# nv-tlabs/NKSR

Hardware: AMD Instinct MI355X
Metric: reconstructed points/sec (solve+mesh) (higher is better)
Workload: dtype f32

## Files before the change

nksr_amd/csrc/fused_sweep.hip:

```cpp
#include "fused_dev.h"
#include <type_traits>

__device__ __forceinline__ int half_lane_i(int v, int l, bool upper) {
    const int lo = __builtin_amdgcn_readlane(v, l), hi = __builtin_amdgcn_readlane(v, 32 + l);
    return upper ? hi : lo;
}
__device__ __forceinline__ float half_lane_f(float v, int l, bool upper) { return __int_as_float(half_lane_i(__float_as_int(v), l, upper)); }

template <bool SETUP> struct FzSets { static constexpr int N = SETUP ? 2 : 1, SECOND = N - 1; };

template <int D, bool SETUP> struct FzStage { static constexpr int CAP0 = SETUP ? 64 : 96, CAP1 = D > 1 ? (SETUP ? 16 : 32) : 1; };
template <int D, bool SETUP> using FzStaged0 = float[FzSets<SETUP>::N][FzStage<D, SETUP>::CAP0 * 27];
template <int D, bool SETUP> using FzStaged1 = float[FzSets<SETUP>::N][FzStage<D, SETUP>::CAP1 * 27];
#define FZ_RCAP 288
template <int D, bool FAC = true> struct FzRecords {
    static constexpr int RS = FZ_RCAP + 4 * FZ_HW;
    float4 fv[FAC ? D * RS : 1], fp[FAC ? RS : 1];
};

template <int D, bool SETUP>
__device__ __forceinline__ void fz_zero_uncovered(const FusedArgs& A, int W0, float* __restrict__ part, float* __restrict__ part2) {
    if (W0 > 0 && threadIdx.x < 32 * D) {
        const int d = threadIdx.x >> 5;
        const int c = A.row_cells[(int64_t)d * A.rows_total + W0 - 1];
        if (c >= 0 && A.nbr32[(int64_t)c * 32 + 29] >= W0) {
            const int64_t blk = (int64_t)A.nbr32[(int64_t)c * 32 + 27] + blockIdx.x;
            part[blk * 32 + (threadIdx.x & 31)] = 0.f;
            if (SETUP) part2[blk * 32 + (threadIdx.x & 31)] = 0.f;
        }
    }
    if (SETUP && A.nnz_counter && threadIdx.x == 0) A.nnz_counter[1 + blockIdx.x] = 0;
}

template <int D, bool SETUP>
__device__ __forceinline__ void fz_flush(const FzStaged0<D, SETUP>& st0, const FzStaged1<D, SETUP>& st1, const int* stf, float* __restrict__ ct,
                                         float* __restrict__ ct2, int cw0, int cw1, int M) {
    constexpr int SECOND = FzSets<SETUP>::SECOND, CAP0 = FzStage<D, SETUP>::CAP0, CAP1 = FzStage<D, SETUP>::CAP1;
    const int t = threadIdx.x;
    const bool l0 = t < CAP0, l1 = !l0 && t < CAP0 + CAP1;
    if ((l0 || l1) && stf[t]) {
        const float* src = l0 ? st0[0] + t * 27 : st1[0] + (t - CAP0) * 27;
        const float* srcb = SETUP ? (l0 ? st0[SECOND] + t * 27 : st1[SECOND] + (t - CAP0) * 27) : nullptr;
        float* dst = ct + (l0 ? cw0 + t : cw1 + (t - CAP0));
        float* dstb = SETUP ? ct2 + (l0 ? cw0 + t : cw1 + (t - CAP0)) : nullptr;
#pragma unroll
        for (int q = 0; q < 27; ++q) {
            dst[(int64_t)q * M] = src[q];
            if (SETUP) dstb[(int64_t)q * M] = srcb[q];
        }
    }
}

struct FzSpline { float a[3], b[3], c[3]; };
__device__ __forceinline__ FzSpline fz_spline_consts(int s) {
    FzSpline q;
    const int o[3] = {s / 9, (s / 3) % 3, s % 3};
#pragma unroll
    for (int ax = 0; ax < 3; ++ax) {
        q.a[ax] = o[ax] == 1 ? 0.75f : 0.f;
        q.b[ax] = o[ax] == 1 ? -1.f : 0.5f;
        q.c[ax] = o[ax] == 0 ? 1.f : (o[ax] == 1 ? 0.5f : 0.f);
    }
    return q;
}
template <bool DER>
__device__ __forceinline__ void fz_axis(float p, float scale, float a, float b, float c, float k, float& w, float& dw) {
    const float u = __builtin_amdgcn_fractf(p * scale);
    const float t = u - c, bt = b * t;
    w = fmaf(bt, t, a);
    if (DER) dw = bt * k;
}
__device__ __forceinline__ float fz_dot4(const float4& a, const float4& b) {
    return fmaf(a.w, b.w, fmaf(a.z, b.z, fmaf(a.y, b.y, a.x * b.x)));
}

template <int D>
__device__ __forceinline__ void fz_stage_records(const FusedArgs& A, int W0, int W1, FzRecords<D>& R) {
    const int nw = W1 - W0 < FZ_RCAP ? W1 - W0 : FZ_RCAP;
    if (nw > 0) {
        const int t0 = threadIdx.x, t1 = threadIdx.x + FZ_BLOCK;
        float4 v0[D + 1], v1[D + 1];
#pragma unroll
        for (int d = 0; d <= D; ++d) {
            const float4* src = (d < D ? A.fac_vec + (int64_t)d * A.rows_total : A.fac_pos) + W0;
            v0[d] = src[t0 < nw ? t0 : nw - 1];
            v1[d] = src[t1 < nw ? t1 : nw - 1];
        }
        const float4 zero = make_float4(0.f, 0.f, 0.f, 0.f);
#pragma unroll
        for (int d = 0; d <= D; ++d) {
            float4* dst = d < D ? R.fv + d * R.RS : R.fp;
            if (t0 < nw + 4 && t0 < FZ_RCAP) dst[t0] = t0 < nw ? v0[d] : zero;
            if (t1 < nw + 4 && t1 < FZ_RCAP) dst[t1] = t1 < nw ? v1[d] : zero;
        }
    }
}

template <int D, bool SETUP>
__device__ __forceinline__ void fz_rebuild_rows(const FusedArgs& A, FzRecords<D>& R, const FzSpline& bq, float4 (&ps)[D], bool live0, const float4& pg,
                                                int r, int W0, int hwi, int s, bool act, int& nt, float (&w)[FZ_TRIP][D]) {
    constexpr int U = FZ_TRIP, RS = FzRecords<D>::RS;
    int rl = r - W0;
    if (rl + U > FZ_RCAP) {
        rl = FZ_RCAP + 4 * hwi;
        if (s < 4) {
            R.fp[rl + s] = A.fac_pos[(int64_t)r + s];
#pragma unroll
            for (int d = 0; d < D; ++d) R.fv[d * RS + rl + s] = A.fac_vec[(int64_t)d * A.rows_total + r + s];
        }
        __builtin_amdgcn_wave_barrier();
    }
    float4 pq[U];
#pragma unroll
    for (int u = 0; u < U; ++u) pq[u] = R.fp[rl + u];
    const bool site = __float_as_int(pq[0].w) == 1;
    const bool q1 = __float_as_int(pq[1].w) == 0, q2 = q1 && __float_as_int(pq[2].w) == 0, q3 = q2 && __float_as_int(pq[3].w) == 0;
    const int np = site ? U : 1 + (q1 ? 1 : 0) + (q2 ? 1 : 0) + (q3 ? 1 : 0);
    nt = nt < np ? nt : np;
    ps[0] = live0 ? pg : make_float4(0.f, 0.f, 0.f, 0.f);
#pragma unroll
    for (int d = 0; d < D; ++d) {
        const float scale = __int_as_float((127 - d) << 23);
        const float k2 = 2.f * A.inv_w0 * scale;
        float4 vq[U];
#pragma unroll
        for (int u = 0; u < U; ++u) vq[u] = R.fv[d * RS + rl + u];
        if (site) {
            float wx, wy, wz, dx, dy, dz;
            fz_axis<true>(pq[0].x, scale, bq.a[0], bq.b[0], bq.c[0], k2, wx, dx);
            fz_axis<true>(pq[0].y, scale, bq.a[1], bq.b[1], bq.c[1], k2, wy, dy);
            fz_axis<true>(pq[0].z, scale, bq.a[2], bq.b[2], bq.c[2], k2, wz, dz);
            const float yz = wy * wz, B = wx * yz;
            const float g = fz_dot4(vq[0], ps[d]);
            w[0][d] = 0.f;
            w[1][d] = fmaf(fz_dot4(vq[1], ps[d]), B, g * (dx * yz));
            w[2][d] = fmaf(fz_dot4(vq[2], ps[d]), B, g * ((wx * wz) * dy));
            w[3][d] = fmaf(fz_dot4(vq[3], ps[d]), B, g * ((wx * wy) * dz));
        } else {
#pragma unroll
            for (int u = 0; u < U; ++u) {
                float wx, wy, wz, unused;
                fz_axis<false>(pq[u].x, scale, bq.a[0], bq.b[0], bq.c[0], 0.f, wx, unused);
                fz_axis<false>(pq[u].y, scale, bq.a[1], bq.b[1], bq.c[1], 0.f, wy, unused);
                fz_axis<false>(pq[u].z, scale, bq.a[2], bq.b[2], bq.c[2], 0.f, wz, unused);
                w[u][d] = fz_dot4(vq[u], ps[d]) * (wx * (wy * wz));
            }
        }
    }
    if (SETUP && A.dense_out) {
#pragma unroll
        for (int d = 0; d < D; ++d)
            if (d >= A.dense_from && act)
#pragma unroll
                for (int u = 0; u < U; ++u)
                    if (u < nt) A.dense_out[((int64_t)(d - A.dense_from) * A.rows_total + r + u) * 27 + s] = w[u][d];
    }
}

template <int MODE, int D, bool FAC>
__global__ void __attribute__((amdgpu_waves_per_eu(FAC ? 3 : (D <= 4 ? 6 : 5)))) __launch_bounds__(FZ_BLOCK) k_fz_cells(FusedArgs A, const float* __restrict__ x, float* __restrict__ part,
                                                      float* __restrict__ part2, float* __restrict__ ct, float* __restrict__ ct2,
                                                      const int* __restrict__ done) {
    if (done && *done) return;
    constexpr bool SETUP = MODE == 1;
    constexpr int U = FZ_TRIP, SECOND = FzSets<SETUP>::SECOND;
    __shared__ float xv[FzSets<SETUP>::N][FZ_HW][D][2][32];
    __shared__ int xm[FZ_HW][D][2];
    __shared__ int xmb[FZ_HW][D][2];
    __shared__ int xbase[FZ_HW][D];
    __shared__ int wnnz[FZ_BLOCK / 64];
    constexpr int CAP0 = FzStage<D, SETUP>::CAP0, CAP1 = FzStage<D, SETUP>::CAP1;
    __shared__ FzStaged0<D, SETUP> st0;
    __shared__ FzStaged1<D, SETUP> st1;
    __shared__ int stf[CAP0 + CAP1];
    __shared__ FzRecords<D, FAC> R;
    for (int i = threadIdx.x; i < CAP0 + CAP1; i += FZ_BLOCK) stf[i] = 0;
    const int W0 = __builtin_amdgcn_readfirstlane(A.item_begin[blockIdx.x * FZ_HW]);
    if (__builtin_amdgcn_readfirstlane(A.item_begin[(blockIdx.x + 1) * FZ_HW]) == W0) {
        fz_zero_uncovered<D, SETUP>(A, W0, part, part2);
        return;
    }
    if constexpr (FAC) {
        const int W1 = __builtin_amdgcn_readfirstlane(A.item_begin[(blockIdx.x + 1) * FZ_HW]);
        if (MODE == 0 && W1 > W0 && fz_seg_done(A, A.item_seg, W0 >> 5)) return;
        fz_stage_records<D>(A, W0, W1, R);
    }
    __syncthreads();
    const int hwi = threadIdx.x >> 5;
    const int item = blockIdx.x * FZ_HW + hwi;
    const int s = threadIdx.x & 31;
    const bool act = s < 27, upper = (threadIdx.x & 32) != 0;
    const int sh = upper ? 32 : 0;
    const int sc = act ? s : 26;
    const int Rb = A.item_begin[item];
    int Re = A.item_begin[item + 1];
    if (MODE == 0 && Re > Rb && fz_seg_done(A, A.item_seg, Rb >> 5)) Re = Rb;
    const int cw0 = __builtin_amdgcn_readfirstlane((int64_t)W0 < A.rows_total ? A.row_cells[W0] : -1);
    const int cw1 = __builtin_amdgcn_readfirstlane((D > 1 && (int64_t)W0 < A.rows_total) ? A.row_cells[A.rows_total + W0] : -1);
    if (s < 2 * D) xm[hwi][s >> 1][s & 1] = -1;
    const int len32 = Re - Rb < 32 ? Re - Rb : 32;
    int cells[D];
    unsigned chg[D > 1 ? D : 2];
    unsigned um = 0;
#pragma unroll
    for (int d = 0; d < D; ++d) {
        cells[d] = s < len32 ? A.row_cells[(int64_t)d * A.rows_total + Rb + s] : -1;
        const int before = __shfl_up(cells[d], 1, 32);
        const unsigned m = (unsigned)(__ballot(s > 0 && s < len32 && cells[d] != before) >> sh);
        if (d > 0) chg[d] = m;
        um |= m;
    }
    um |= 1u;
    unsigned inside = 0;
    float P[FzSets<SETUP>::N][D], xs[D];
    bool have[D];
#pragma unroll
    for (int d = 0; d < D; ++d) { P[0][d] = 0.f; P[SECOND][d] = 0.f; xs[d] = 0.f; have[d] = false; }
    auto enter = [&](int d, int nbv) {
        const int first = __shfl(nbv, 28, 32), last = __shfl(nbv, 29, 32);
        if (s == 27) xbase[hwi][d] = nbv;
        inside = (inside & ~(3u << (2 * d))) | ((first >= Rb ? 1u : 0u) << (2 * d)) | ((last < Re ? 2u : 0u) << (2 * d));
    };
    auto finish = [&](int d, int cell, float p, float p2) {
        const int rel = d == 0 ? cell - cw0 : cell - cw1;
        if (d == 0 && cw0 >= 0 && (unsigned)rel < (unsigned)CAP0) {
            if (act) { st0[0][rel * 27 + s] = p; if (SETUP) st0[SECOND][rel * 27 + s] = p2; }
            if (s == 0) stf[rel] = 1;
        } else if (d == 1 && cw1 >= 0 && (unsigned)rel < (unsigned)CAP1) {
            if (act) { st1[0][rel * 27 + s] = p; if (SETUP) st1[SECOND][rel * 27 + s] = p2; }
            if (s == 0) stf[CAP0 + rel] = 1;
        } else if (act) {
            ct[(int64_t)s * A.M + cell] = p;
            if (SETUP) ct2[(int64_t)s * A.M + cell] = p2;
        }
    };
    auto emit = [&](int d, int cell, float p, float p2) {
        const unsigned f = (inside >> (2 * d)) & 3u;
        if (f == 3u) {
            finish(d, cell, p, p2);
        } else {
            const int k = (int)(f & 1u);
            xv[0][hwi][d][k][s] = p;
            if (SETUP) xv[SECOND][hwi][d][k][s] = p2;
            if (s == 0) { xm[hwi][d][k] = cell | ((f & 2u) ? (1 << 30) : 0); xmb[hwi][d][k] = xbase[hwi][d]; }
        }
    };
    auto unit_end = [&](int p) {
        const unsigned after = um & ~((2u << p) - 1u);
        return after ? Rb + (int)__builtin_ctz(after) : Re;
    };
    bool work = Rb < Re;
    int pos = 0, r = Rb, uend = unit_end(0);
    const float* wp[D];
#pragma unroll
    for (int d = 0; d < D; ++d) wp[d] = FAC ? nullptr : A.rows_all + (int64_t)d * A.rows_total * 27 + sc;
    int c0 = __shfl(cells[0], 0, 32);
    int line0;
    const float4 zero4 = make_float4(0.f, 0.f, 0.f, 0.f);
    float4 ps[D];
    {
        int cd[D], nb0[D];
        float x0[D];
        float4 p0[D];
#pragma unroll
        for (int d = 0; d < D; ++d) {
            cd[d] = __shfl(cells[d], 0, 32);
            nb0[d] = A.nbr32[(int64_t)(cd[d] >= 0 ? cd[d] : 0) * 32 + s];
        }
#pragma unroll
        for (int d = 1; d < D; ++d) {
            x0[d] = MODE == 0 ? x[(act && nb0[d] >= 0) ? nb0[d] : 0] : 0.f;
            if (FAC) p0[d] = A.psi_all[(act && nb0[d] >= 0) ? nb0[d] : 0];
        }
        line0 = nb0[0];
#pragma unroll
        for (int d = 1; d < D; ++d) {
            have[d] = work && cd[d] >= 0;
            enter(d, nb0[d]);
            xs[d] = (have[d] && act && nb0[d] >= 0) ? x0[d] : 0.f;
            if (FAC) ps[d] = (have[d] && act && nb0[d] >= 0) ? p0[d] : zero4;
        }
        if (FAC) ps[0] = zero4;
    }
    const FzSpline bq = fz_spline_consts(sc);
    int nnz = 0;
    while (__any(work)) {
        float w[U][D];
        if (!FAC) {
#pragma unroll
            for (int u = 0; u < U; ++u)
#pragma unroll
                for (int d = 0; d < D; ++d) w[u][d] = *(wp[d] + ((int64_t)r + u) * 27);
        }
        const float xg = MODE == 0 ? x[(act && line0 >= 0) ? line0 : 0] : 0.f;
        float4 pg = zero4;
        if (FAC) pg = A.psi_all[(act && line0 >= 0) ? line0 : 0];
        float tg[U];
        if (MODE == 1) {
#pragma unroll
            for (int u = 0; u < U; ++u) tg[u] = A.targets_all ? A.targets_all[r + u] : 0.f;
        }
        const int npos = uend - Rb;
        const int cn = __shfl(cells[0], npos & 31, 32);
        const int line0n = A.nbr32[(int64_t)((uend < Re && cn >= 0) ? cn : 0) * 32 + s];
        int nt = work ? (uend - r < U ? uend - r : U) : 0;
        if constexpr (FAC) {
            fz_rebuild_rows<D, SETUP>(A, R, bq, ps, c0 >= 0 && act && line0 >= 0, pg, r, W0, hwi, s, act, nt, w);
        }
        const float x0 = (c0 >= 0 && act && line0 >= 0) ? xg : 0.f;
        float t[U];
        if (MODE == 0) {
            float prod[U];
#pragma unroll
            for (int u = 0; u < U; ++u) {
                prod[u] = w[u][0] * x0;
#pragma unroll
                for (int d = 1; d < D; ++d) prod[u] = fmaf(w[u][d], xs[d], prod[u]);
            }
            const float rs = half_sum4(prod[0], prod[1], prod[2], prod[3], s);
#pragma unroll
            for (int u = 0; u < U; ++u) t[u] = u < nt ? half_lane_f(rs, 8 * u, upper) : 0.f;
        } else {
#pragma unroll
            for (int u = 0; u < U; ++u) {
                const bool ok = u < nt && act;
                t[u] = u < nt ? tg[u] : 0.f;
#pragma unroll
                for (int d = 0; d < D; ++d) { w[u][d] = ok ? w[u][d] : 0.f; nnz += w[u][d] != 0.f ? 1 : 0; }
            }
        }
#pragma unroll
        for (int u = 0; u < U; ++u)
#pragma unroll
            for (int d = 0; d < D; ++d) {
                P[0][d] = fmaf(w[u][d], t[u], P[0][d]);
                if (SETUP) P[SECOND][d] = fmaf(w[u][d], w[u][d], P[SECOND][d]);
            }
        r += nt;
        if (work && r >= uend) {
            if (c0 >= 0) finish(0, c0, P[0][0], P[SECOND][0]);
            P[0][0] = 0.f;
            if (SETUP) P[SECOND][0] = 0.f;
            work = uend < Re;
            if (work) {
                pos = npos;
                c0 = cn;
                line0 = line0n;
                uend = unit_end(pos);
#pragma unroll
                for (int d = 1; d < D; ++d)
                    if ((chg[d] >> pos) & 1u) {
                        const int before = __shfl(cells[d], (pos + 31) & 31, 32);
                        if (have[d]) emit(d, before, P[0][d], P[SECOND][d]);
                        P[0][d] = 0.f;
                        if (SETUP) P[SECOND][d] = 0.f;
                        xs[d] = 0.f;
                        if (FAC) ps[d] = zero4;
                        const int cd = __shfl(cells[d], pos, 32);
                        have[d] = cd >= 0;
                        if (have[d]) {
                            const int nbv = A.nbr32[(int64_t)cd * 32 + s];
                            enter(d, nbv);
                            if (MODE == 0 && act && nbv >= 0) xs[d] = x[nbv];
                            if (FAC && act && nbv >= 0) ps[d] = A.psi_all[nbv];
                        }
                    }
            }
        }
    }
#pragma unroll
    for (int d = 1; d < D; ++d)
        if (have[d]) emit(d, __shfl(cells[d], pos, 32), P[0][d], P[SECOND][d]);
    if (SETUP && A.nnz_counter) {
#pragma unroll
        for (int o = 32; o > 0; o >>= 1) nnz += __shfl_xor(nnz, o);
        if ((threadIdx.x & 63) == 0) wnnz[threadIdx.x >> 6] = nnz;
    }
    __syncthreads();
    if (SETUP && A.nnz_counter && threadIdx.x == 0) {
        unsigned long long tot = 0;
#pragma unroll
        for (int q = 0; q < FZ_BLOCK / 64; ++q) tot += (unsigned long long)wnnz[q];
        A.nnz_counter[1 + blockIdx.x] = tot;
    }
#pragma unroll
    for (int d = 1; d < D; ++d)
#pragma unroll
        for (int k = 0; k < 2; ++k) {
            const int e = xm[hwi][d][k];
            if (e < 0) continue;
            const int c = e & ~(1 << 30);
            const bool ends = (e >> 30) & 1;
            bool later = false;
            if (!ends)
                for (int h = hwi + 1; h < FZ_HW; ++h) later = later || (xm[h][d][0] >= 0 && (xm[h][d][0] & ~(1 << 30)) == c);
            if (later) continue;
            int h0 = hwi;
            bool started = k == 1;
            while (!started && h0 > 0) {
                --h0;
                started = xm[h0][d][1] >= 0 && (xm[h0][d][1] & ~(1 << 30)) == c;
            }
            float acc = 0.f, acc2 = 0.f;
            for (int h = h0; h <= hwi; ++h) {
                const int kk = (h == h0 && started) ? 1 : 0;
                const int eh = h == hwi ? e : xm[h][d][kk];
                if (eh < 0 || (eh & ~(1 << 30)) != c) continue;
                acc += xv[0][h][d][kk][s];
                if (SETUP) acc2 += xv[SECOND][h][d][kk][s];
            }
            if (started && ends) {
                finish(d, c, acc, acc2);
            } else {
                const int base = xmb[hwi][d][k];
                part[((int64_t)base + blockIdx.x) * 32 + s] = acc;
                if (SETUP) part2[((int64_t)base + blockIdx.x) * 32 + s] = acc2;
            }
        }
    __syncthreads();
    fz_flush<D, SETUP>(st0, st1, stf, ct, ct2, cw0, cw1, A.M);
}

template <int MAX, class F>
static inline void fz_with_depth(int depth, F&& f) {
    if constexpr (MAX > 1) {
        if (depth < MAX) return fz_with_depth<MAX - 1>(depth, f);
    }
    f(std::integral_constant<int, MAX>{});
}

template <int MODE>
void fz_sweep(const FusedArgs& A, const float* x, const FusedWork& w, const int* done, hipStream_t st) {
    if (A.hw_total <= 0) return;
    const dim3 grid(nksr_blocks((int64_t)A.hw_total, FZ_HW)), blk(FZ_BLOCK);
    fz_with_depth<NKSR_MAX_DEPTH>(A.depth, [&](auto depth) {
        constexpr int D = decltype(depth)::value;
        if (A.fac_vec) hipLaunchKernelGGL((k_fz_cells<MODE, D, true>), grid, blk, 0, st, A, x, w.part, w.part2, w.ct, w.ct2, done);
        else hipLaunchKernelGGL((k_fz_cells<MODE, D, false>), grid, blk, 0, st, A, x, w.part, w.part2, w.ct, w.ct2, done);
    });
}
template void fz_sweep<0>(const FusedArgs&, const float*, const FusedWork&, const int*, hipStream_t);
template void fz_sweep<1>(const FusedArgs&, const float*, const FusedWork&, const int*, hipStream_t);
```

Baseline: 33.25 million.

## Prefetch row weight tiles through a register ring staged via LDS in fz_cells

For the non-factored path, each half-wave now loads contiguous 16-byte pieces covering a trip's rows into a two-deep register ring, one trip ahead. It scatters them into an LDS tile and reads the per-lane weights back, replacing strided scalar global loads. Neighbour lines, x stencil values and targets are also fetched one trip ahead. Occupancy hints are lowered (waves_per_eu 6/5 to 4/3) to leave room for the extra live registers. The costs are more register pressure, more LDS use and explicit waitcnt/wave barriers, plus some risk in the row-advance bookkeeping at unit boundaries.

```diff
diff --git a/nksr_amd/csrc/fused_sweep.hip b/nksr_amd/csrc/fused_sweep.hip
--- a/nksr_amd/csrc/fused_sweep.hip
+++ b/nksr_amd/csrc/fused_sweep.hip
@@ -17,6 +17,18 @@
     static constexpr int RS = FZ_RCAP + 4 * FZ_HW;
     float4 fv[FAC ? D * RS : 1], fp[FAC ? RS : 1];
 };
+
+#define FZ_PIECES 28
+#define FZ_RING 2
+typedef float fz_piece_t __attribute__((ext_vector_type(4)));
+template <int D, bool ON = true> struct FzRowTiles { fz_piece_t v[ON ? FZ_HW * D * FZ_PIECES : 1]; };
+__device__ __forceinline__ const fz_piece_t* fz_row_piece(const float* rows, int64_t first, int s) {
+    const float* b = rows + first;
+    const int o4 = (int)(reinterpret_cast<uintptr_t>(b) & 12u);
+    int off = 16 * s < 428 + o4 ? 16 * s : 428 + o4;
+    off &= ~15;
+    return reinterpret_cast<const fz_piece_t*>(b + ((off - o4) >> 2));
+}
 
 template <int D, bool SETUP>
 __device__ __forceinline__ void fz_zero_uncovered(const FusedArgs& A, int W0, float* __restrict__ part, float* __restrict__ part2) {
@@ -158,7 +170,7 @@
 }
 
 template <int MODE, int D, bool FAC>
-__global__ void __attribute__((amdgpu_waves_per_eu(FAC ? 3 : (D <= 4 ? 6 : 5)))) __launch_bounds__(FZ_BLOCK) k_fz_cells(FusedArgs A, const float* __restrict__ x, float* __restrict__ part,
+__global__ void __attribute__((amdgpu_waves_per_eu(FAC ? 3 : (D <= 4 ? 4 : 3)))) __launch_bounds__(FZ_BLOCK) k_fz_cells(FusedArgs A, const float* __restrict__ x, float* __restrict__ part,
                                                       float* __restrict__ part2, float* __restrict__ ct, float* __restrict__ ct2,
                                                       const int* __restrict__ done) {
     if (done && *done) return;
@@ -174,6 +186,7 @@
     __shared__ FzStaged1<D, SETUP> st1;
     __shared__ int stf[CAP0 + CAP1];
     __shared__ FzRecords<D, FAC> R;
+    __shared__ FzRowTiles<D, !FAC> rt;
     for (int i = threadIdx.x; i < CAP0 + CAP1; i += FZ_BLOCK) stf[i] = 0;
     const int W0 = __builtin_amdgcn_readfirstlane(A.item_begin[blockIdx.x * FZ_HW]);
     if (__builtin_amdgcn_readfirstlane(A.item_begin[(blockIdx.x + 1) * FZ_HW]) == W0) {
@@ -251,9 +264,34 @@
     };
     bool work = Rb < Re;
     int pos = 0, r = Rb, uend = unit_end(0);
-    const float* wp[D];
-#pragma unroll
-    for (int d = 0; d < D; ++d) wp[d] = FAC ? nullptr : A.rows_all + (int64_t)d * A.rows_total * 27 + sc;
+    constexpr int RING = FAC ? 1 : FZ_RING;
+    fz_piece_t pc0[D], pc1[D], pc2[D];
+    int rp0 = 0, rp1 = 0, rp2 = 0;
+    int rq = Rb, uq = uend, pq = 0;
+    int lq0 = 0, lq1 = 0, lq2 = 0;
+    if ((int64_t)rq >= A.rows_total) rq = (int)A.rows_total - 1;
+    auto fetch_nbr = [&](int& row) {
+        const int cq = __shfl(cells[0], pq & 31, 32);
+        row = A.nbr32[(int64_t)(cq >= 0 ? cq : 0) * 32 + s];
+    };
+    auto fetch = [&](fz_piece_t (&p)[D], int& first) {
+        first = rq;
+#pragma unroll
+        for (int d = 0; d < D; ++d) p[d] = *fz_row_piece(A.rows_all + (int64_t)d * A.rows_total * 27, (int64_t)rq * 27, s);
+    };
+    auto advance = [&]() {
+        const int rn = rq + U < uq ? rq + U : uq;
+        if (rn < Re) {
+            if (rn >= uq) { pq = uq - Rb; uq = unit_end(pq); }
+            rq = rn;
+        }
+    };
+    float* const tile = reinterpret_cast<float*>(rt.v) + hwi * D * (4 * FZ_PIECES);
+    if constexpr (!FAC) {
+        fetch_nbr(lq0); fetch(pc0, rp0);
+        if constexpr (RING > 1) { advance(); fetch_nbr(lq1); fetch(pc1, rp1); }
+        if constexpr (RING > 2) { advance(); fetch_nbr(lq2); fetch(pc2, rp2); }
+    }
     int c0 = __shfl(cells[0], 0, 32);
     int line0;
     const float4 zero4 = make_float4(0.f, 0.f, 0.f, 0.f);
@@ -282,28 +320,67 @@
         }
         if (FAC) ps[0] = zero4;
     }
+    float xq0 = 0.f, xq1 = 0.f, xq2 = 0.f, tq0[U], tq1[U], tq2[U];
+    if constexpr (!FAC) {
+        static_assert(FZ_RING >= 2, "a trip's x stencil and targets are fetched into the ring's next entry");
+        if (MODE == 0) xq0 = x[(act && lq0 >= 0) ? lq0 : 0];
+#pragma unroll
+        for (int u = 0; u < U; ++u) tq0[u] = (MODE == 1 && A.targets_all) ? A.targets_all[r + u] : 0.f;
+    }
     const FzSpline bq = fz_spline_consts(sc);
     int nnz = 0;
-    while (__any(work)) {
+    auto trip = [&](auto phase) {
+        constexpr int ph = decltype(phase)::value;
+        fz_piece_t (&pc)[D] = ph == 0 ? pc0 : (ph == 1 ? pc1 : pc2);
+        int& rp = ph == 0 ? rp0 : (ph == 1 ? rp1 : rp2);
         float w[U][D];
-        if (!FAC) {
-#pragma unroll
-            for (int u = 0; u < U; ++u)
-#pragma unroll
-                for (int d = 0; d < D; ++d) w[u][d] = *(wp[d] + ((int64_t)r + u) * 27);
-        }
-        const float xg = MODE == 0 ? x[(act && line0 >= 0) ? line0 : 0] : 0.f;
+        float xg = 0.f, tg[U];
         float4 pg = zero4;
-        if (FAC) pg = A.psi_all[(act && line0 >= 0) ? line0 : 0];
-        float tg[U];
-        if (MODE == 1) {
-#pragma unroll
-            for (int u = 0; u < U; ++u) tg[u] = A.targets_all ? A.targets_all[r + u] : 0.f;
-        }
         const int npos = uend - Rb;
         const int cn = __shfl(cells[0], npos & 31, 32);
-        const int line0n = A.nbr32[(int64_t)((uend < Re && cn >= 0) ? cn : 0) * 32 + s];
         int nt = work ? (uend - r < U ? uend - r : U) : 0;
+        int line0n;
+        if constexpr (FAC) {
+            if (MODE == 0) xg = x[(act && line0 >= 0) ? line0 : 0];
+            pg = A.psi_all[(act && line0 >= 0) ? line0 : 0];
+            if (MODE == 1) {
+#pragma unroll
+                for (int u = 0; u < U; ++u) tg[u] = A.targets_all ? A.targets_all[r + u] : 0.f;
+            }
+            line0n = A.nbr32[(int64_t)((uend < Re && cn >= 0) ? cn : 0) * 32 + s];
+        } else {
+            float& xnext = ph + 1 == RING ? xq0 : (ph == 0 ? xq1 : xq2);
+            float (&tnext)[U] = ph + 1 == RING ? tq0 : (ph == 0 ? tq1 : tq2);
+            const int lnext = ph + 1 == RING ? lq0 : (ph == 0 ? lq1 : lq2);
+            line0 = ph == 0 ? lq0 : (ph == 1 ? lq1 : lq2);
+            line0n = line0;
+            advance();
+            fetch_nbr(ph == 0 ? lq0 : (ph == 1 ? lq1 : lq2));
+            if (MODE == 0) xnext = x[(act && lnext >= 0) ? lnext : 0];
+            if (MODE == 1) {
+#pragma unroll
+                for (int u = 0; u < U; ++u) tnext[u] = A.targets_all ? A.targets_all[r + nt + u] : 0.f;
+            }
+            xg = ph == 0 ? xq0 : (ph == 1 ? xq1 : xq2);
+#pragma unroll
+            for (int u = 0; u < U; ++u) tg[u] = ph == 0 ? tq0[u] : (ph == 1 ? tq1[u] : tq2[u]);
+        }
+        if constexpr (!FAC) {
+            const unsigned ob = (unsigned)(reinterpret_cast<uintptr_t>(A.rows_all) >> 2);
+#pragma unroll
+            for (int d = 0; d < D; ++d)
+                if (s < FZ_PIECES) rt.v[(hwi * D + d) * FZ_PIECES + s] = pc[d];
+            __builtin_amdgcn_wave_barrier();
+#pragma unroll
+            for (int d = 0; d < D; ++d) {
+                const unsigned o = (ob + (unsigned)(((int64_t)d * A.rows_total + rp) * 27)) & 3u;
+                const float* q = tile + d * (4 * FZ_PIECES) + o + sc;
+#pragma unroll
+                for (int u = 0; u < U; ++u) w[u][d] = q[27 * u];
+            }
+            __builtin_amdgcn_wave_barrier();
+            fetch(pc, rp);
+        }
         if constexpr (FAC) {
             fz_rebuild_rows<D, SETUP>(A, R, bq, ps, c0 >= 0 && act && line0 >= 0, pg, r, W0, hwi, s, act, nt, w);
         }
@@ -363,11 +440,19 @@
                             enter(d, nbv);
                             if (MODE == 0 && act && nbv >= 0) xs[d] = x[nbv];
                             if (FAC && act && nbv >= 0) ps[d] = A.psi_all[nbv];
+                            if constexpr (!FAC) __builtin_amdgcn_s_waitcnt(0x0F70);
                         }
                     }
             }
         }
-    }
+    };
+    if constexpr (!FAC) __builtin_amdgcn_s_waitcnt(0x0F70);
+    while (__any(work)) {
+        trip(std::integral_constant<int, 0>{});
+        if constexpr (RING > 1) trip(std::integral_constant<int, 1>{});
+        if constexpr (RING > 2) trip(std::integral_constant<int, 2>{});
+    }
+    static_assert(RING <= 3, "the row loop names the ring's registers one by one");
 #pragma unroll
     for (int d = 1; d < D; ++d)
         if (have[d]) emit(d, __shfl(cells[d], pos, 32), P[0][d], P[SECOND][d]);
```

Measured after the change: 29.63 million. 0.891x the previous value.
